# lixinustc/KVQ-Challenge-CVPR-NTIRE2024

Measured on AMD Instinct MI355X. Metric: videos/sec (8-frag x 32 x 224 x 224), higher is better.
Workload: dtype bf16

## Files before the change

### include/kvq_hip.h

```cpp
#ifndef KVQ_HIP_H
#define KVQ_HIP_H

#include <stddef.h>
#include <stdint.h>

#ifdef __cplusplus
extern "C" {
#endif

#define KVQ_ABI_VERSION 31
#define KVQ_MAX_STAGES 4

typedef enum { KVQ_DT_BF16 = 0, KVQ_DT_FP16 = 1 } KvqDtype;

typedef enum {
  KVQ_OK = 0,
  KVQ_ERR_NULL = -1,
  KVQ_ERR_SHAPE = -2,
  KVQ_ERR_UNSUPPORTED = -3,
  KVQ_ERR_WORKSPACE = -4,
  KVQ_ERR_HIP = -5
} KvqStatus;

int kvq_abi_version(void);
// ... 275 lines not shown

int kvq_window_attention(const uint16_t* qkv, const int32_t* tok, const float* rpb, const float* fpb,
                         const float* bias_pack, int table_len, int center, int BW, int nW, int N, int num_heads, int use_mask,
                         int dtype, uint16_t* out, void* stream);

size_t kvq_attn_bias32_bytes(int n_types, int N, int num_heads);
int kvq_attn_bias32_build(const int32_t* tok, const float* rpb, const float* fpb, int table_len, int center,
                          int n_types, int N, int num_heads, int use_mask, void* out, float* max_abs, void* stream);
typedef struct {
  const uint16_t* qkv;
  const void* bias_dense;
  int32_t n_types, BW, nW, N, num_heads, dtype;
  uint16_t* out;
  const uint32_t* tile_skip;
  int32_t dsplit_from;
  const uint16_t* x_ln;
  const uint16_t* w_qkv;
  const float* b_qkv;
  float q_scale;
  const uint32_t* pad_mask;
} KvqAttnDenseArgs;
int kvq_window_attention32(const KvqAttnDenseArgs* host_args, void* stream);
int kvq_window_attention32_ranges(const KvqAttnDenseArgs* host_args, const uint8_t* ranges, void* stream);
int kvq_attn32_row_order(const int32_t* tok_host, int n_windows, int N, int32_t* order);
int kvq_attn32_key_ranges(const int32_t* tok_host, int n_windows, int N, int use_mask, uint8_t* ranges);

int kvq_patch_im2col(const float* x, int B, int Cin, int T, int H, int W, int pd, int ph, int pw,
                     int dtype, uint16_t* out, void* stream);

int kvq_vqa_head(const float* feat, int B, int L, int C, int64_t stride_b, int64_t stride_l,
                 int64_t stride_c, const float* w1t, const float* w1, const float* b1, int hidden, const float* w2,
                 const float* b2, float* scratch, float* score, void* stream);

int kvq_vqa_head_map(const float* feat, int B, int L, int C, int64_t stride_b, int64_t stride_l, int64_t stride_c,
                     const float* w1t, const float* w1, const float* b1, int hidden, const float* w2, const float* b2,
                     int D, float* tok_map, float* depth_score, float* score, void* stream);

typedef struct {
  const KvqFragmentSource* src;
  int32_t T, D, Hf, Wf;
  int32_t cell;
  const float* tok_map;
  float* heat;
  float* cover;
  uint8_t* overlay;
  int32_t ov_depth[16];
  int32_t n_ov;
  const float* range;
// ... 275 lines not shown
```

### kvq-challenge-cvpr-ntire2024_amd/_abi.py

```python
from __future__ import annotations

import ctypes as C
import os
from typing import Optional

from . import _build

MAX_STAGES = 4
K_NAMES = ["im2col", "layernorm", "gemm_qkv", "attn", "gemm_proj", "gemm_fc1", "gemm_fc2", "gemm_merge",
           "gemm_embed", "tail", "embed", "merge"]
K_COUNT = len(K_NAMES)

EPI_BIAS_BF16, EPI_GELU_BF16, EPI_QKV_BF16, EPI_RESID_F32, EPI_STORE_F32, EPI_RELU_BF16, EPI_QGELU_BF16, EPI_RESID_SCALE_F32 = range(8)
DT_BF16, DT_FP16 = 0, 1
ABI_VERSION = 31


def dtype_code(dt) -> int:
    import torch
    is_int = isinstance(dt, int) and not isinstance(dt, bool)
    if (is_int and dt == DT_FP16) or (not is_int and dt in (torch.float16, "fp16", "float16")):
        return DT_FP16
    if (is_int and dt == DT_BF16) or (not is_int and dt in (torch.bfloat16, "bf16", "bfloat16")):
        return DT_BF16
# ... 240 lines not shown
    "kvq_patch_embed_fragments_supported": (i32, [C.POINTER(KvqFragmentSource), i32, i32, i32, i32, i32, i32]),
    "kvq_patch_embed_pack_bytes": (sz, [i32, i32]),
    "kvq_patch_embed_pack": (i32, [p_void, p_void, p_void, p_void, i32, i32, p_void, p_void]),
    "kvq_patch_embed": (i32, [C.POINTER(KvqPatchEmbedArgs), p_void]),
    "kvq_patch_merge_supported": (i32, [i32]),
    "kvq_patch_merge_pack_bytes": (sz, [i32]),
    "kvq_patch_merge_pack": (i32, [p_void, p_void, p_void, i32, i32, p_void, p_void]),
    "kvq_patch_merge": (i32, [C.POINTER(KvqPatchMergeArgs), p_void]),
    "kvq_block_tail_supported": (i32, [i32, i32]),
    "kvq_block_tail_pack_bytes": (sz, [i32, i32]),
    "kvq_block_tail_pack": (i32, [p_void, p_void, p_void, p_void, p_void, p_void, p_void, p_void, i32, i32, p_void,
                                  p_void]),
    "kvq_block_tail_qkv_pack_bytes": (sz, [i32, i32]),
    "kvq_block_tail_qkv_pack": (i32, [p_void, i32, i32, p_void, p_void]),
    "kvq_block_tail": (i32, [C.POINTER(KvqBlockTailArgs), p_void]),
    "kvq_window_attention": (i32, [p_void, p_void, p_void, p_void, p_void, i32, i32, i32, i32, i32, i32, i32, i32, p_void,
                                   p_void]),
    "kvq_attn_bias32_bytes": (sz, [i32, i32, i32]),
    "kvq_attn_bias32_build": (i32, [p_void, p_void, p_void, i32, i32, i32, i32, i32, i32, p_void, p_void, p_void]),
    "kvq_window_attention32": (i32, [C.POINTER(KvqAttnDenseArgs), p_void]),
    "kvq_window_attention32_ranges": (i32, [C.POINTER(KvqAttnDenseArgs), p_void, p_void]),
    "kvq_attn32_row_order": (i32, [p_void, i32, i32, p_void]),
    "kvq_attn32_key_ranges": (i32, [p_void, i32, i32, i32, p_void]),
    "kvq_swin3d_bias_dense_bytes": (sz, [p_void, i32]),
    "kvq_swin3d_bias_dense_build": (i32, [p_void, i32, p_void, p_void, p_void, p_void, p_void]),
    "kvq_patch_im2col": (i32, [p_void, i32, i32, i32, i32, i32, i32, i32, i32, i32, p_void, p_void]),
    "kvq_vqa_head": (i32, [p_void, i32, i32, i32, i64, i64, i64, p_void, p_void, p_void, i32, p_void, p_void, p_void,
                           p_void, p_void]),
    "kvq_vqa_head_map": (i32, [p_void, i32, i32, i32, i64, i64, i64, p_void, p_void, p_void, i32, p_void, p_void, i32, p_void,
                               p_void, p_void, p_void]),
    "kvq_quality_paint_supported": (i32, [C.POINTER(KvqFragmentSource), i32, i32, i32, i32, i32]),
    "kvq_quality_paint": (i32, [C.POINTER(KvqQualityPaintArgs), p_void]),
    "kvq_quality_paint_regions_supported": (i32, [C.POINTER(KvqFragmentSource), i32, i32, i32, i32, i32, i32, i32, i32]),
    "kvq_quality_paint_regions": (i32, [C.POINTER(KvqQualityPaintRegionArgs), p_void]),
    "kvq_vqa_head_classes": (i32, [p_void, i32, i32, i32, i64, i64, i64, p_void, p_void, i32, p_void, p_void, i32, i32, p_void,
                                   p_void, p_void]),
    "kvq_simple_vqa_head": (i32, [p_void, i32, i32, i32, p_void, p_void, i32, p_void, p_void, p_void, p_void,
                                  p_void]),
    "kvq_resize_bilinear": (i32, [p_void, i32, i32, i32, i32, i32, i32, i32, i32, i32, i32, i32, i32, C.POINTER(f32),
                                  C.POINTER(f32), p_void, p_void]),
    "kvq_resize_bilinear_aa": (i32, [p_void, i32, i32, i32, i32, i32, i32, i32, i32, i32, i32, i32, i32, C.POINTER(f32),
                                     C.POINTER(f32), p_void, p_void]),
    "kvq_resize_aa_taps": (i32, [i32, i32, C.POINTER(i32), p_void, p_void, p_void]),
    "kvq_resize_pil_taps": (i32, [i32, i32, C.POINTER(i32), p_void, p_void, p_void]),
    "kvq_resize_pil_supported": (i32, [i32] * 6),
    "kvq_resize_pil": (i32, [p_void, i32, i32, i32, i32, i32, i32, p_void, p_void, p_void, p_void, p_void, p_void, p_void, p_void, i64, i64,
# ... 118 lines not shown
```

### kvq-challenge-cvpr-ntire2024_amd/csrc/attn32.hip

```cpp
#include <stdlib.h>

#include "common.hpp"

#ifndef A32_ABL
#define A32_ABL 0
#endif
#ifndef A32_SUM
#define A32_SUM 0
#endif
#if (A32_ABL & 2)
#define A32_EXP(x) ((x) * 0.001f + 1.0f)
#else
#define A32_EXP(x) __builtin_amdgcn_exp2f(x)
#endif

#ifdef KVQ_DIAG
#define A32_DIAG_FLAG(x) (x)
#else
#define A32_DIAG_FLAG(x) false
#endif

namespace kvq {

constexpr int A32_KB = 13;
// ... 187 lines not shown
      ls = E::dot2(P[cur][i], one2, ls);
      ls1 = E::dot2(P[cur][i + 1], one2, ls1);
    }
#endif
    if (t + 1 < T1) {
      __builtin_amdgcn_sched_group_barrier(0x002, 16, 1);
      __builtin_amdgcn_sched_group_barrier(0x008, 1, 1);
      __builtin_amdgcn_sched_group_barrier(0x002, 12, 1);
      __builtin_amdgcn_sched_group_barrier(0x008, 1, 1);
    }
    __builtin_amdgcn_sched_barrier(0);
  }
  ls += ls1;
  if (A32_SUM == 1) ls = (lv0[0] + lv0[1]) + (lv1[0] + lv1[1]);
  ls = a32_pair_sum(ls);
  a32_finish<E>(O, ls, orow, store);
#undef A32_NR
}

struct Attn32Params {
  const uint16_t* qkv;
  const u32x4* image;
  int BW, nW, N, nH, n_types, qsplit;
  uint16_t* out;
  const uint32_t* tile_skip;
  int dsplit_from;
  const uint8_t* ranges;
  const uint16_t* x_ln;
  const uint16_t* w_qkv;
  const float* b_qkv;
  float q_scale;
  uint16_t* q_out;
  const uint32_t* pad_mask;
  bool no_q_store;
  bool image_one;
};

template <typename E, int KS>
__device__ __forceinline__ void a32_fused_qkv(const Attn32Params& p, unsigned char* slot, int bw, int h, int N) {
  using V8 = typename E::v8;
  const int tid = threadIdx.x, lane = tid & 63, j = lane & 15, g = lane >> 4;
  const int wave = __builtin_amdgcn_readfirstlane(tid >> 6);
  const int C = KS * 32;
  const size_t Mtot = (size_t)p.BW * N;
  const uint16_t* xw = p.x_ln + (size_t)bw * N * C;
  uint16_t* qo = p.q_out + ((size_t)h * Mtot + (size_t)bw * N) * 32;
// ... 49 lines not shown
}

enum { kAllKeys = 0, kDepthSplit = 1, kRanges = 2 };
template <typename E, bool FUSED, int MODE, bool SHORT = false>
__global__ __launch_bounds__(A32_WAVES * 64, 3) __attribute__((amdgpu_waves_per_eu(3, 3))) void window_attention32_kernel(Attn32Params p) {
  fp16_saturate_mode();
  extern __shared__ __attribute__((aligned(16))) unsigned char smem[];
  int* ticket = reinterpret_cast<int*>(smem + A32_OFF_CTR);
  using V8 = typename E::v8;
  const int nclip = p.BW / p.nW, nrep = p.nW / p.n_types, npair = p.n_types * p.nH, per_pair = nclip * nrep * p.qsplit;
  const int xcd = blockIdx.x & 7, slot_i = blockIdx.x >> 3;
  int pair, clip, rep, part;
  if (FUSED) {
    const int per_type = p.nH * nclip * nrep, wt_ = (slot_i / per_type) * 8 + xcd, sub = slot_i % per_type;
    if (wt_ >= p.n_types) return;
    const int h_ = sub % p.nH, rest = sub / p.nH;
    pair = wt_ * p.nH + h_; clip = rest % nclip; rep = rest / nclip; part = 0;
  } else {
    const int sub = slot_i % per_pair;
    pair = (slot_i / per_pair) * 8 + xcd;
    clip = sub % nclip; rep = (sub / nclip) % nrep; part = sub / (nclip * nrep);
  }
  if (pair >= npair) return;
  const int wt = pair / p.nH, h = pair - wt * p.nH, w = rep * p.n_types + wt, bw = clip * p.nW + w;
  const int tid = threadIdx.x, lane = tid & 63, N = p.N, nqb = (N + 31) >> 5;
  const int wave = __builtin_amdgcn_readfirstlane(tid >> 6);
  const size_t Mtot = (size_t)p.BW * N;
  const int C = p.nH * 32;
  const uint16_t* Qg = p.qkv + ((size_t)h * Mtot + (size_t)bw * N) * 32;

  int range_of_lane = 0;
  if (MODE == kRanges) {
    const uint8_t* rg = p.ranges + ((size_t)w * A32_KB + min(lane, A32_KB - 1)) * 2;
    const int first = rg[0], need = (int)rg[1] - first + 1;
    const int len = need <= 4 ? 4 : need <= 7 ? 7 : A32_KB;
    range_of_lane = min(first, A32_KB - len) | (len << 8);
  }
  if (tid < 64) *reinterpret_cast<u32x4*>(smem + A32_OFF_ZERO + tid * 16) = (u32x4){0u, 0u, 0u, 0u};
  if (FUSED) {
    for (int i = tid; i < (A32_ROWS - N) * 8; i += A32_WAVES * 64)
      *reinterpret_cast<u32x4*>(smem + (i & 4 ? A32_K_BYTES : 0) + (N + (i >> 3)) * 64 + (i & 3) * 16) = (u32x4){0u, 0u, 0u, 0u};
    a32_fused_qkv<E, 3>(p, smem, bw, h, N);
  } else {
    const uint16_t* Kg = p.qkv + ((size_t)(1 * p.nH + h) * Mtot + (size_t)bw * N) * 32;
    const uint16_t* Vg = p.qkv + ((size_t)(2 * p.nH + h) * Mtot + (size_t)bw * N) * 32;
    const __amdgpu_buffer_rsrc_t rk = __builtin_amdgcn_make_buffer_rsrc(const_cast<uint16_t*>(Kg), 0, N * 64, 0x00020000);
    const __amdgpu_buffer_rsrc_t rv = __builtin_amdgcn_make_buffer_rsrc(const_cast<uint16_t*>(Vg), 0, N * 64, 0x00020000);
// ... 22 lines not shown
    __syncthreads();
  }

  const int q = lane & 31, hi = lane >> 5;
  const uint32_t skip = p.tile_skip ? p.tile_skip[w] : 0u;
  const bool dsplit = MODE == kDepthSplit && p.dsplit_from >= 0 && w >= p.dsplit_from;
  auto key_range = [&](int qb, int& t0, int& len) __attribute__((always_inline)) {
    t0 = 0; len = A32_KB;
    if (MODE == kDepthSplit && dsplit && qb != 6) { t0 = qb < 6 ? 0 : 6; len = 7; }
    if (MODE == kRanges) {
      const int r = __builtin_amdgcn_readlane(range_of_lane, qb);
      t0 = r & 0xff; len = r >> 8;
    }
  };
  auto take = [&]() -> int {
    int qb_;
    do {
      qb_ = 0;
      if (lane == 0) qb_ = atomicAdd(ticket, 1);
      qb_ = __builtin_amdgcn_readfirstlane(qb_);
    } while (qb_ < q_hi && ((skip >> (2 * qb_)) & 1u) && (((skip >> (2 * qb_ + 1)) & 1u) || 32 * qb_ + 16 >= N));
    return qb_;
  };
  const u32x4* img = p.image + (size_t)(A32_DIAG_FLAG(p.image_one) ? h : pair) * nqb * (A32_KB * 128) + lane;
  struct Req { V8 qf0, qf1; u32x4 pre[2]; int t0, len; };
  auto request = [&](int qb, Req& r) __attribute__((always_inline)) {
    const int qrow = min(32 * qb + q, N - 1);
    r.qf0 = *reinterpret_cast<const V8*>(Qg + (size_t)qrow * 32 + 8 * hi);
    r.qf1 = *reinterpret_cast<const V8*>(Qg + (size_t)qrow * 32 + 16 + 8 * hi);
    if (!FUSED && p.pad_mask && ((p.pad_mask[(size_t)w * A32_KB + qb] >> q) & 1u)) {
      r.qf0 = __builtin_bit_cast(V8, (u32x4){0u, 0u, 0u, 0u});
      r.qf1 = r.qf0;
    }
    key_range(min(qb, nqb - 1), r.t0, r.len);
    const u32x4* bd = img + (size_t)min(qb, nqb - 1) * (A32_KB * 128) + r.t0 * 128;
    r.pre[0] = bd[0]; r.pre[1] = bd[64];
  };
  auto run = [&](int qb, const Req& r) __attribute__((always_inline)) {
    const u32x4* bd = img + (size_t)qb * (A32_KB * 128);
    uint16_t* orow = p.out + ((size_t)bw * N + 32 * qb + q) * C + h * 32;
    const bool store = 32 * qb + q < N;
    const int zero = A32_OFF_ZERO >> 4;
    const int t0 = MODE == kRanges ? r.t0 : 0;
    if (MODE != kAllKeys && r.len == 7) {
      if (r.t0 == A32_KB - 7) a32_qblock<E, 7, true, SHORT>(smem, zero, bd, A32_KB - 7, r.qf0, r.qf1, r.pre, orow, store);
      else a32_qblock<E, 7, false>(smem, zero, bd, t0, r.qf0, r.qf1, r.pre, orow, store);
    } else if (MODE == kRanges && r.len == 4) {
// ... 144 lines not shown
extern "C" int kvq_attn32_key_ranges(const int32_t* tok_host, int n_windows, int N, int use_mask, uint8_t* ranges) {
  using namespace kvq;
  KVQ_REQUIRE(tok_host && ranges, KVQ_ERR_NULL, "kvq_attn32_key_ranges: NULL pointer");
  KVQ_REQUIRE(n_windows > 0 && N >= 1 && N <= 400, KVQ_ERR_SHAPE, "kvq_attn32_key_ranges: bad shape n_windows=%d N=%d", n_windows, N);
  const int nkb = (N + 31) / 32;
  for (int w = 0; w < n_windows; ++w) {
    const int32_t* tk = tok_host + (size_t)w * N * 2;
    for (int qb = 0; qb < A32_KB; ++qb) {
      int first = 0, last = nkb - 1;
      if (use_mask && qb < nkb) {
        bool in_block[256] = {false};
        for (int qq = 32 * qb; qq < N && qq < 32 * qb + 32; ++qq) in_block[(tk[2 * qq + 1] >> 16) & 0xff] = true;
        first = nkb; last = -1;
        for (int key = 0; key < N; ++key)
          if (in_block[(tk[2 * key + 1] >> 16) & 0xff]) { first = first < (key >> 5) ? first : key >> 5; last = key >> 5; }
      }
      ranges[((size_t)w * A32_KB + qb) * 2] = (uint8_t)first;
      ranges[((size_t)w * A32_KB + qb) * 2 + 1] = (uint8_t)last;
    }
  }
  return KVQ_OK;
}

static int window_attention32(const char* who, const KvqAttnDenseArgs* a, const uint8_t* ranges, void* stream) {
  using namespace kvq;
  KVQ_REQUIRE(a && a->qkv && a->bias_dense && a->out, KVQ_ERR_NULL, "%s: NULL pointer", who);
  const int BW = a->BW, nW = a->nW, N = a->N, num_heads = a->num_heads, n_types = a->n_types;
  KVQ_REQUIRE(BW > 0 && nW > 0 && BW % nW == 0 && num_heads > 0 && n_types > 0 && nW % n_types == 0, KVQ_ERR_SHAPE,
              "%s: bad shape BW=%d nW=%d n_types=%d nH=%d", who, BW, nW, n_types, num_heads);
  KVQ_REQUIRE(N >= 1 && N <= 400, KVQ_ERR_UNSUPPORTED, "%s: window of %d tokens unsupported (1..400)", who, N);
  KVQ_REQUIRE(((size_t)a->bias_dense & 15) == 0, KVQ_ERR_SHAPE, "%s: the bias image must be 16-byte aligned", who);
  KVQ_REQUIRE_OPERAND(who, a->dtype);
  KVQ_REQUIRE(a->dsplit_from < 0 || (N == 392 && a->dsplit_from < nW), KVQ_ERR_UNSUPPORTED,
              "%s: depth-split windows need the (8,7,7) window (N = 392); got N=%d from=%d", who, N, a->dsplit_from);
  const int units = BW * num_heads, nqb = (N + 31) / 32;
  int qsplit = units >= 768 ? 1 : 768 / units;
  const int qsplit_max = latency_mode() ? 4 : 1;
  qsplit = qsplit > qsplit_max ? qsplit_max : qsplit;
  qsplit = qsplit > nqb ? nqb : qsplit;
  Attn32Params p{a->qkv, (const u32x4*)a->bias_dense, BW, nW, N, num_heads, n_types, qsplit, a->out, a->tile_skip,
                     a->dsplit_from < 0 ? -1 : a->dsplit_from};
#ifdef KVQ_DIAG
  { static const bool one = getenv("KVQ_IMAGE_ONE_TYPE") && atoi(getenv("KVQ_IMAGE_ONE_TYPE")) == 1; p.image_one = one; }
  { static const bool nq = getenv("KVQ_NO_Q_STORE") && atoi(getenv("KVQ_NO_Q_STORE")) == 1; p.no_q_store = nq; }
#endif
  if (a->pad_mask) {
    KVQ_REQUIRE(a->b_qkv && !a->x_ln, KVQ_ERR_NULL, "%s: pad_mask needs b_qkv (and excludes the fused projection)", who);
    p.pad_mask = a->pad_mask; p.b_qkv = a->b_qkv;
  }
  if (a->x_ln) {
    const int C = 32 * num_heads;
    KVQ_REQUIRE(a->w_qkv && a->b_qkv, KVQ_ERR_NULL, "%s: x_ln without w_qkv / b_qkv", who);
    KVQ_REQUIRE(C == 96, KVQ_ERR_UNSUPPORTED, "%s: the fused qkv projection is built for C = 96 (got %d)", who, C);
    KVQ_REQUIRE((((size_t)a->x_ln | (size_t)a->w_qkv | (size_t)a->b_qkv) & 15) == 0, KVQ_ERR_SHAPE,
                "%s: x_ln / w_qkv / b_qkv must be 16-byte aligned", who);
    p.qsplit = 1;
    p.x_ln = a->x_ln; p.w_qkv = a->w_qkv; p.b_qkv = a->b_qkv; p.q_scale = a->q_scale; p.q_out = const_cast<uint16_t*>(a->qkv);
  }
  if (ranges) {
    KVQ_REQUIRE(a->dsplit_from < 0 && !a->pad_mask, KVQ_ERR_UNSUPPORTED, "%s: key ranges exclude dsplit_from and pad_mask (un-padded partitions only)", who);
    p.ranges = ranges;
  }
  return with_operand(a->dtype, [&](auto e) { return launch_attn32_e<decltype(e)>(p, (hipStream_t)stream); });
}

extern "C" int kvq_window_attention32(const KvqAttnDenseArgs* a, void* stream) {
  return window_attention32("kvq_window_attention32", a, nullptr, stream);
}

extern "C" int kvq_window_attention32_ranges(const KvqAttnDenseArgs* a, const uint8_t* ranges, void* stream) {
  KVQ_REQUIRE(ranges, KVQ_ERR_NULL, "kvq_window_attention32_ranges: NULL ranges");
  return window_attention32("kvq_window_attention32_ranges", a, ranges, stream);
}
```

### kvq-challenge-cvpr-ntire2024_amd/csrc/plan.hip

```cpp
#include <math.h>
#include <stdlib.h>
#include <string.h>

#include <vector>

#include "common.hpp"
#include "tail.hpp"

#ifdef KVQ_DIAG
static int skip_mask() {
  static const int m = [] {
    const int v = getenv("KVQ_SKIP") ? atoi(getenv("KVQ_SKIP")) : 0;
    if (v) fprintf(stderr, "libkvq_hip (KVQ_DIAG build): KVQ_SKIP=%d leaves launch families out - scores are GARBAGE, timing only\n", v);
    return v;
  }();
  return m;
}
#else
static constexpr int skip_mask() { return 0; }
#endif

namespace kvq {

struct StageGeom {
  int D, H, W, C, nH, depth;
  int L;
  int ws[3], ss[3];
  int Dp, Hp, Wp, nW, N, Lp;
  bool shifted_any;
  int32_t* d_src[2];
  int32_t* d_pad[2];
  int32_t* d_skip[2];
  int32_t* d_padmask[2];
  int32_t* d_dst[2];
  int32_t* d_tok[2];
  uint8_t* d_ranges[2];
  int32_t* d_merge;
  int Dn, Hn, Wn;
};

struct ProfEvent {
  int kind, variant;
  double flops, bytes;
  hipEvent_t a, b;
};

}

struct KvqSwinPlan {
  KvqSwinCfg cfg;
  int B, T, H, W, dtype;
  int D0, H0, W0, K0;
  std::vector<kvq::StageGeom> st;
  std::vector<void*> owned;
  size_t ws_bytes;
  size_t off_x0, off_x1, off_ln, off_big, off_o, off_sk, sk_bytes;
  size_t region_bytes[6];
  unsigned char* run_ws;
// ... 116 lines not shown
    if (!pad.empty()) {
      rc = upload(pl, pad, &g.d_pad[par]);
      if (rc) return rc;
      if (g.N <= 13 * 32) {
        std::vector<int32_t> pm((size_t)g.nW * 13, 0);
        for (int i : pad) pm[(size_t)(i / g.N) * 13 + ((i % g.N) >> 5)] |= (int32_t)(1u << ((i % g.N) & 31));
        rc = upload(pl, pm, &g.d_padmask[par]);
        if (rc) return rc;
      }
      std::vector<int32_t> skip((size_t)g.nW, 0);
      bool any = false;
      for (int wv = 0; wv < g.nW; ++wv)
        for (int t = 0; t * 16 < g.N && t < 32; ++t) {
          bool all_pad = true;
          for (int q = t * 16; q < g.N && q < t * 16 + 16; ++q) all_pad = all_pad && src[(size_t)wv * g.N + q] < 0;
          if (all_pad) { skip[wv] |= (int32_t)(1u << t); any = true; }
        }
      if (any) {
        rc = upload(pl, skip, &g.d_skip[par]);
        if (rc) return rc;
      }
    }
  }
  return upload(pl, tok, &g.d_tok[par]);
}

static int build_merge_map(KvqSwinPlan* pl, StageGeom& g) {
  g.Dn = g.D; g.Hn = (g.H + 1) / 2; g.Wn = (g.W + 1) / 2;
  std::vector<int32_t> m((size_t)g.Dn * g.Hn * g.Wn * 4);
  size_t r = 0;
  for (int d = 0; d < g.D; ++d)
    for (int h2 = 0; h2 < g.Hn; ++h2)
      for (int w2 = 0; w2 < g.Wn; ++w2, ++r) {
        const int hh[4] = {2 * h2, 2 * h2 + 1, 2 * h2, 2 * h2 + 1};
        const int wv[4] = {2 * w2, 2 * w2, 2 * w2 + 1, 2 * w2 + 1};
        for (int p = 0; p < 4; ++p)
          m[4 * r + p] = (hh[p] < g.H && wv[p] < g.W) ? (d * g.H + hh[p]) * g.W + wv[p] : -1;
      }
  return upload(pl, m, &g.d_merge);
}

static size_t align_up(size_t v) { return (v + 255) & ~(size_t)255; }

}

extern "C" int kvq_swin3d_plan_create(const KvqSwinCfg* cfg, int B, int T, int H, int W, int dtype,
                                      KvqSwinPlan** out) {
// ... 96 lines not shown
  for (int i = 0; i < pl->cfg.num_stages; ++i) {
    const StageGeom& g = pl->st[i];
    if (block < k + g.depth) {
      *stage = i;
      *par = ((block - k) & 1) && g.shifted_any ? 1 : 0;
      return block >= k;
    }
    k += g.depth;
  }
  return false;
}
}

namespace kvq {
static int bias_types(const StageGeom& g, int par) { return par == 0 ? g.nW / (g.Dp / g.ws[0]) : g.nW; }
constexpr float kQScale = 0.17677669529663687f;
constexpr float kQScaleLog2 = 0.17677669529663687f * 1.4426950408889634f;
}

extern "C" size_t kvq_swin3d_bias_dense_bytes(const KvqSwinPlan* pl, int block) {
  int i = 0, par = 0;
  if (!pl || !kvq::locate_block(pl, block, &i, &par)) return 0;
  const kvq::StageGeom& g = pl->st[i];
  return kvq_attn_bias32_bytes(kvq::bias_types(g, par), g.N, g.nH);
}

extern "C" int kvq_swin3d_bias_dense_build(const KvqSwinPlan* pl, int block, const float* rpb, const float* fpb, void* out,
                                           float* max_abs, void* stream) {
  using namespace kvq;
  int i = 0, par = 0;
  KVQ_REQUIRE(pl && rpb && out, KVQ_ERR_NULL, "kvq_swin3d_bias_dense_build: NULL pointer");
  KVQ_REQUIRE(locate_block(pl, block, &i, &par), KVQ_ERR_SHAPE, "kvq_swin3d_bias_dense_build: no block %d", block);
  const StageGeom& g = pl->st[i];
  return kvq_attn_bias32_build(g.d_tok[par], rpb, pl->cfg.frag_bias[i] ? fpb : nullptr, pl->table_len, pl->center,
                               bias_types(g, par), g.N, g.nH, par, out, max_abs, stream);
}

extern "C" int kvq_swin3d_profile(KvqSwinPlan* pl, int enable) {
  using namespace kvq;
  KVQ_REQUIRE(pl, KVQ_ERR_NULL, "kvq_swin3d_profile: NULL");
  pl->profile = enable != 0;
  pl->ev_used = 0;
  return KVQ_OK;
}

extern "C" int kvq_swin3d_profile_read(KvqSwinPlan* pl, KvqProfRecord* out, int max_records, int* n_records) {
  using namespace kvq;
  KVQ_REQUIRE(pl && out && n_records, KVQ_ERR_NULL, "kvq_swin3d_profile_read: NULL");
  int n = 0;
  for (size_t i = 0; i < pl->ev_used && n < max_records; ++i, ++n) {
    ProfEvent& e = pl->events[i];
    KVQ_CHECK_HIP(hipEventSynchronize(e.b));
    float t = 0.f;
    KVQ_CHECK_HIP(hipEventElapsedTime(&t, e.a, e.b));
    out[n].kind = e.kind; out[n].variant = e.variant; out[n].ms = t; out[n].flops = e.flops; out[n].bytes = e.bytes;
  }
  *n_records = n;
  pl->ev_used = 0;
// ... 196 lines not shown
    const int C = g.C;
    const float qs = bw.bias_dense ? kQScaleLog2 : kQScale;
    if (t.ln1 != kFromProducer)
      KVQ_TRY(ln(pl, st, cur, t.ln1 == kLnTokens ? nullptr : g.d_src[t.par], 1, g.L, t.ln1 == kLnTokens ? g.L : g.Lp, C, bw.norm1_w,
                 bw.norm1_b, bln, nullptr, s.x16[t.i]));
    if (t.qkv == kQkvGemm)
      KVQ_TRY_UNLESS(8 | (t.i == last ? 32 : 0), gemm(pl, st, KVQ_K_GEMM_QKV, bln, bw.qkv_w, bw.qkv_b, B * g.Lp, 3 * C, C, KVQ_EPI_QKV_BF16, bbig, nullptr, g.nH, qs));
    if (t.qkv == kQkvGemmPadded)
      KVQ_TRY(gemm(pl, st, KVQ_K_GEMM_QKV, bln, bw.qkv_w, bw.qkv_b, B * g.L, 3 * C, C, KVQ_EPI_QKV_BF16, bbig, nullptr, g.nH,
                   qs, g.d_dst[t.par], g.L, g.Lp));
    if (t.fill_pad) KVQ_TRY(kvq_qkv_fill_pad(bbig, bw.qkv_b, g.d_pad[t.par], g.Lp - g.L, B, g.Lp, g.nH, qs, pl->dtype, st));
    return KVQ_OK;
  };

  auto attention = [&](const BlockStep& t, const StageGeom& g, const KvqSwinBlockW& bw) -> int {
    const int C = g.C, M = B * g.Lp;
    if (!t.dense) {
      Bracket br(pl, st, KVQ_K_ATTN, (cfg.frag_bias[t.i] ? 2 : 0) + t.par, 4.0 * M * g.N * C, 2.0 * 4.0 * M * C);
      return kvq_window_attention(bbig, g.d_tok[t.par], bw.rpb_table, cfg.frag_bias[t.i] ? bw.fpb_table : nullptr, bw.bias_pack,
                                  pl->table_len, pl->center, B * g.nW, g.nW, g.N, g.nH, t.par, pl->dtype, bo, st);
    }
    const bool fq = t.qkv == kQkvInAttn;
    Bracket br(pl, st, KVQ_K_ATTN, 4 + t.par, 4.0 * M * g.N * C + (fq ? 6.0 * M * C * C : 0.0),
               (fq ? 2.0 * 2.0 * M * C + 6.0 * C * C : 2.0 * 4.0 * M * C) + (double)kvq_swin3d_bias_dense_bytes(pl, t.blk));
    KvqAttnDenseArgs aa{};
    aa.qkv = bbig; aa.bias_dense = bw.bias_dense; aa.n_types = bias_types(g, t.par); aa.BW = B * g.nW; aa.nW = g.nW; aa.N = g.N;
    aa.num_heads = g.nH; aa.dtype = pl->dtype; aa.out = bo; aa.tile_skip = (const uint32_t*)g.d_skip[t.par]; aa.dsplit_from = t.dsplit_from;
    if (fq) { aa.x_ln = bln; aa.w_qkv = bw.qkv_w; aa.b_qkv = bw.qkv_b; aa.q_scale = kQScaleLog2; }
    if (t.pad_mask) { aa.pad_mask = (const uint32_t*)g.d_padmask[t.par]; aa.b_qkv = bw.qkv_b; }
    if (g.d_ranges[t.par]) KVQ_TRY_UNLESS(1 | (t.i == last ? 32 : 0), kvq_window_attention32_ranges(&aa, g.d_ranges[t.par], st));
    else KVQ_TRY_UNLESS(1 | (t.i == last ? 32 : 0), kvq_window_attention32(&aa, st));
    return KVQ_OK;
  };

  auto tail = [&](const BlockStep& t, const StageGeom& g, const KvqSwinBlockW& bw) -> int {
    const int C = g.C, M = B * g.Lp, ML = B * g.L, hidden = cfg.mlp_ratio * C, skip_last = t.i == last ? 32 : 0;
    if (t.fused_tail) {
      const bool e1 = t.emit == kEmitLn1, eq = t.emit == kEmitQkv, x16 = s.x16[t.i];
      KvqBlockTailArgs ta{};
      ta.attn = bo; ta.x = cur; ta.scatter_map = g.d_src[t.par]; ta.map_rows = g.Lp; ta.out_rows = g.L;
      ta.M = M; ta.C = C; ta.hidden = hidden; ta.pack = bw.tail_pack; ta.eps = 1e-5f; ta.dtype = pl->dtype; ta.x_f16 = x16 ? 1 : 0;
      if (g.Lp != g.L) ta.attn_gather = g.d_dst[t.par];
      if (t.emit != kEmitNone) {
        const KvqSwinBlockW& nb = w->blocks[t.blk + 1];
        ta.next_norm_w = nb.norm1_w; ta.next_norm_b = nb.norm1_b; ta.next_dst = g.d_dst[t.npar]; ta.next_rows = g.Lp;
        if (eq) { ta.next_qkv_pack = nb.qkv_pack; ta.next_qkv_b = nb.qkv_b; ta.qkv_out = bbig; ta.q_scale = kQScaleLog2; ta.num_heads = g.nH; }
        else ta.next_ln = bln;
      }
      Bracket br(pl, st, KVQ_K_TAIL, kvq::tailmm_geometry_code(C, hidden) * 1000 + (C / 32) * 10 + t.emit, 2.0 * M * C * C + 4.0 * (double)ML * C * hidden + (eq ? 6.0 * M * C * C : 0.0),
                 (double)M * C * 2.0 + (double)ML * C * ((x16 ? 4.0 : 8.0) + (e1 ? 2.0 : 0.0) + (eq ? 6.0 : 0.0)));
      KVQ_TRY_UNLESS(C <= 192 ? 2 : 4, block_tail_launch(&ta, range_of(t.i), st));
      return KVQ_OK;
    }
    if (g.Lp != g.L) {
// ... 117 lines not shown
```

### kvq-challenge-cvpr-ntire2024_amd/kernels.py

```python
from __future__ import annotations

import ctypes as C
from typing import Optional, Sequence

import torch

from . import _abi
from ._abi import check, current_stream, dtype_code, lib, ptr, stream_of
from ._prepared import to_operand

HALF_TYPES = (torch.float16, torch.bfloat16)


def _need_gpu(*ts):
    for t in ts:
        if t is not None and not t.is_cuda:
            raise _abi.KvqError("kvq_amd kernels need tensors on a HIP device (no CPU fallback exists)")


def device_name() -> str:
    buf = C.create_string_buffer(256)
    check(lib().kvq_device_name(buf, 256), "kvq_device_name")
    return buf.value.decode()

# ... 156 lines not shown
    check(lib().kvq_window_attention(ptr(qkv), ptr(tok), ptr(rpb), ptr(fpb), ptr(bias_pack), rpb.shape[0], center, BW, nW, N, nH,
                                     int(use_mask), dtype_code(qkv.dtype), ptr(out), current_stream()),
          "kvq_window_attention")
    return out


LOG2E = 1.4426950408889634


def attn_bias32(tok: torch.Tensor, rpb: torch.Tensor, fpb: Optional[torch.Tensor], center: int, nW: int, N: int, use_mask: bool):
    _need_gpu(tok, rpb, fpb)
    nH = rpb.shape[1]
    out = torch.empty(lib().kvq_attn_bias32_bytes(nW, N, nH), dtype=torch.uint8, device=rpb.device)
    big = torch.zeros(1, dtype=torch.float32, device=rpb.device)
    check(lib().kvq_attn_bias32_build(ptr(tok), ptr(rpb), ptr(fpb), rpb.shape[0], center, nW, N, nH, int(use_mask),
                                      ptr(out), ptr(big), current_stream()), "kvq_attn_bias32_build")
    out.max_abs_bias = big
    return out


def window_attention32(qkv: torch.Tensor, image: torch.Tensor, nW: int, N: int, n_types: Optional[int] = None,
                       tile_skip: Optional[torch.Tensor] = None, out: Optional[torch.Tensor] = None, dsplit_from: int = -1,
                       x_ln: Optional[torch.Tensor] = None, w_qkv: Optional[torch.Tensor] = None, b_qkv: Optional[torch.Tensor] = None,
                       q_scale: float = 1.0, pad_mask: Optional[torch.Tensor] = None, ranges: Optional[torch.Tensor] = None):
    _need_gpu(qkv, image, tile_skip, out, pad_mask, ranges)
    assert qkv.dtype in HALF_TYPES and qkv.is_contiguous()
    nH = qkv.shape[1]
    BW = qkv.shape[2] // N
    if out is None:
        out = torch.empty(BW * N, nH * 32, dtype=qkv.dtype, device=qkv.device)
    a = _abi.KvqAttnDenseArgs()
    a.qkv, a.bias_dense, a.n_types, a.BW, a.nW, a.N, a.num_heads = ptr(qkv), ptr(image), nW if n_types is None else n_types, BW, nW, N, nH
    a.dtype, a.out, a.tile_skip, a.dsplit_from = dtype_code(qkv.dtype), ptr(out), ptr(tile_skip), dsplit_from
    if x_ln is not None:
        _need_gpu(x_ln, w_qkv, b_qkv)
        assert x_ln.dtype == qkv.dtype == w_qkv.dtype and x_ln.is_contiguous() and w_qkv.is_contiguous() and b_qkv.dtype == torch.float32
        a.x_ln, a.w_qkv, a.b_qkv, a.q_scale = ptr(x_ln), ptr(w_qkv), ptr(b_qkv), q_scale
    if pad_mask is not None:
        _need_gpu(b_qkv)
        assert pad_mask.dtype == torch.int32 and pad_mask.is_contiguous() and (b_qkv is None or b_qkv.dtype == torch.float32)
        a.pad_mask, a.b_qkv = ptr(pad_mask), ptr(b_qkv)
    if ranges is not None:
        assert ranges.dtype == torch.uint8 and ranges.is_contiguous() and ranges.numel() == nW * 26
        check(lib().kvq_window_attention32_ranges(C.byref(a), ptr(ranges), current_stream()), "kvq_window_attention32_ranges")
        return out
    check(lib().kvq_window_attention32(C.byref(a), current_stream()), "kvq_window_attention32")
    return out


def attn32_row_order(tok, n_windows: int, N: int):
    import numpy as np
    tok = np.ascontiguousarray(np.asarray(tok, dtype=np.int32).reshape(n_windows * N, 2))
    order = np.empty((n_windows, N), np.int32)
    check(lib().kvq_attn32_row_order(tok.ctypes.data, n_windows, N, order.ctypes.data), "kvq_attn32_row_order")
    return order


def attn32_key_ranges(tok, n_windows: int, N: int, use_mask: bool):
    import numpy as np
    tok = np.ascontiguousarray(np.asarray(tok, dtype=np.int32).reshape(n_windows * N, 2))
    ranges = np.empty((n_windows, 13, 2), np.uint8)
    check(lib().kvq_attn32_key_ranges(tok.ctypes.data, n_windows, N, int(use_mask), ranges.ctypes.data), "kvq_attn32_key_ranges")
    return ranges


def patch_im2col(x: torch.Tensor, patch: Sequence[int], out_dtype=torch.float16):
    _need_gpu(x)
    assert x.dtype == torch.float32 and x.is_contiguous()
    B, Cin, T, H, W = x.shape
    pd, ph, pw = patch
    D, Hh, Ww = -(-T // pd), -(-H // ph), -(-W // pw)
    out = torch.empty(B * D * Hh * Ww, Cin * pd * ph * pw, dtype=out_dtype, device=x.device)
    check(lib().kvq_patch_im2col(ptr(x), B, Cin, T, H, W, pd, ph, pw, dtype_code(out_dtype), ptr(out),
                                 current_stream()), "kvq_patch_im2col")
    return out


def vqa_head(feat: torch.Tensor, w1, b1, w2, b2, w1t=None, return_map=False):
    _need_gpu(feat, w1, b1, w2, b2, w1t)
    assert feat.dtype == torch.float32 and feat.dim() == 5
    B, Cc, D, H, W = feat.shape
    L = D * H * W
    sb, sc, sd, sh, sw = feat.stride()
    if not (sh == W * sw and sd == H * sh):
        feat = feat.contiguous()
        sb, sc, sd, sh, sw = feat.stride()
# ... 1301 lines not shown
```

Baseline: 439.5.

## Deduplicate identical attention bias images across window types and balance slot order

At plan time, window types whose token-to-bias key patterns are identical after normalising the fragment offset are grouped, so the dense attention bias image is built and stored only once per distinct pattern. A type table maps each work pair to its real window type and canonical image, and duplicated types are interleaved across eight slots so that blocks sharing an image are spread out. This shrinks the bias buffer and the memory traffic and cache footprint it causes in the attention kernel. The cost is one extra table load per block and more complex host-side planning.

```diff
diff --git a/include/kvq_hip.h b/include/kvq_hip.h
--- a/include/kvq_hip.h
+++ b/include/kvq_hip.h
@@ -321,8 +321,10 @@
 } KvqAttnDenseArgs;
 int kvq_window_attention32(const KvqAttnDenseArgs* host_args, void* stream);
 int kvq_window_attention32_ranges(const KvqAttnDenseArgs* host_args, const uint8_t* ranges, void* stream);
+int kvq_window_attention32_types(const KvqAttnDenseArgs* host_args, const uint8_t* ranges, const int32_t* type_tab, void* stream);
 int kvq_attn32_row_order(const int32_t* tok_host, int n_windows, int N, int32_t* order);
 int kvq_attn32_key_ranges(const int32_t* tok_host, int n_windows, int N, int use_mask, uint8_t* ranges);
+int kvq_attn32_image_types(const int32_t* tok_host, int n_types, int N, int32_t* canon, int32_t* slots, int32_t* n_images);
 
 int kvq_patch_im2col(const float* x, int B, int Cin, int T, int H, int W, int pd, int ph, int pw,
                      int dtype, uint16_t* out, void* stream);
diff --git a/kvq-challenge-cvpr-ntire2024_amd/_abi.py b/kvq-challenge-cvpr-ntire2024_amd/_abi.py
--- a/kvq-challenge-cvpr-ntire2024_amd/_abi.py
+++ b/kvq-challenge-cvpr-ntire2024_amd/_abi.py
@@ -286,6 +286,8 @@
     "kvq_window_attention32_ranges": (i32, [C.POINTER(KvqAttnDenseArgs), p_void, p_void]),
     "kvq_attn32_row_order": (i32, [p_void, i32, i32, p_void]),
     "kvq_attn32_key_ranges": (i32, [p_void, i32, i32, i32, p_void]),
+    "kvq_window_attention32_types": (i32, [C.POINTER(KvqAttnDenseArgs), p_void, p_void, p_void]),
+    "kvq_attn32_image_types": (i32, [p_void, i32, i32, p_void, p_void, p_void]),
     "kvq_swin3d_bias_dense_bytes": (sz, [p_void, i32]),
     "kvq_swin3d_bias_dense_build": (i32, [p_void, i32, p_void, p_void, p_void, p_void, p_void]),
     "kvq_patch_im2col": (i32, [p_void, i32, i32, i32, i32, i32, i32, i32, i32, i32, p_void, p_void]),
diff --git a/kvq-challenge-cvpr-ntire2024_amd/csrc/attn32.hip b/kvq-challenge-cvpr-ntire2024_amd/csrc/attn32.hip
--- a/kvq-challenge-cvpr-ntire2024_amd/csrc/attn32.hip
+++ b/kvq-challenge-cvpr-ntire2024_amd/csrc/attn32.hip
@@ -1,4 +1,8 @@
 #include <stdlib.h>
+
+#include <algorithm>
+#include <map>
+#include <vector>
 
 #include "common.hpp"
 
@@ -233,6 +237,7 @@
   const uint16_t* qkv;
   const u32x4* image;
   int BW, nW, N, nH, n_types, qsplit;
+  const int32_t* type_tab;
   uint16_t* out;
   const uint32_t* tile_skip;
   int dsplit_from;
@@ -328,7 +333,10 @@
     clip = sub % nclip; rep = (sub / nclip) % nrep; part = sub / (nclip * nrep);
   }
   if (pair >= npair) return;
-  const int wt = pair / p.nH, h = pair - wt * p.nH, w = rep * p.n_types + wt, bw = clip * p.nW + w;
+  const int wp = pair / p.nH, h = pair - wp * p.nH;
+  int wt = wp, im = wp;
+  if (p.type_tab) { const int e = p.type_tab[wp]; wt = e & 0xffff; im = e >> 16; }
+  const int w = rep * p.n_types + wt, bw = clip * p.nW + w;
   const int tid = threadIdx.x, lane = tid & 63, N = p.N, nqb = (N + 31) >> 5;
   const int wave = __builtin_amdgcn_readfirstlane(tid >> 6);
   const size_t Mtot = (size_t)p.BW * N;
@@ -397,7 +405,7 @@
     } while (qb_ < q_hi && ((skip >> (2 * qb_)) & 1u) && (((skip >> (2 * qb_ + 1)) & 1u) || 32 * qb_ + 16 >= N));
     return qb_;
   };
-  const u32x4* img = p.image + (size_t)(A32_DIAG_FLAG(p.image_one) ? h : pair) * nqb * (A32_KB * 128) + lane;
+  const u32x4* img = p.image + (size_t)(A32_DIAG_FLAG(p.image_one) ? h : im * p.nH + h) * nqb * (A32_KB * 128) + lane;
   struct Req { V8 qf0, qf1; u32x4 pre[2]; int t0, len; };
   auto request = [&](int qb, Req& r) __attribute__((always_inline)) {
     const int qrow = min(32 * qb + q, N - 1);
@@ -588,7 +596,42 @@
   return KVQ_OK;
 }
 
-static int window_attention32(const char* who, const KvqAttnDenseArgs* a, const uint8_t* ranges, void* stream) {
+extern "C" int kvq_attn32_image_types(const int32_t* tok_host, int n_types, int N, int32_t* canon, int32_t* slots, int32_t* n_images) {
+  KVQ_REQUIRE(tok_host && canon && slots && n_images, KVQ_ERR_NULL, "kvq_attn32_image_types: NULL pointer");
+  KVQ_REQUIRE(n_types > 0 && N >= 1, KVQ_ERR_SHAPE, "kvq_attn32_image_types: bad shape n_types=%d N=%d", n_types, N);
+  std::map<std::vector<int32_t>, int> seen;
+  std::vector<std::vector<int>> members;
+  std::vector<int32_t> key((size_t)N * 2);
+  for (int t = 0; t < n_types; ++t) {
+    const int32_t* tk = tok_host + (size_t)t * N * 2;
+    int fh0 = 255, fw0 = 255;
+    for (int n = 0; n < N; ++n) { fh0 = std::min(fh0, tk[2 * n + 1] & 0xff); fw0 = std::min(fw0, (tk[2 * n + 1] >> 8) & 0xff); }
+    for (int n = 0; n < N; ++n) { key[2 * n] = tk[2 * n]; key[2 * n + 1] = tk[2 * n + 1] - fh0 - (fw0 << 8); }
+    const auto it = seen.emplace(key, (int)members.size());
+    if (it.second) members.emplace_back();
+    canon[t] = it.first->second;
+    members[canon[t]].push_back(t);
+  }
+  *n_images = (int32_t)members.size();
+  for (int t = 0; t < n_types; ++t) slots[t] = t;
+  if ((int)members.size() == n_types) return KVQ_OK;
+  std::vector<int> by_size(members.size());
+  for (size_t i = 0; i < by_size.size(); ++i) by_size[i] = (int)i;
+  std::stable_sort(by_size.begin(), by_size.end(), [&](int a, int b) { return members[a].size() > members[b].size(); });
+  int room[8], fill[8] = {0};
+  for (int c = 0; c < 8; ++c) room[c] = n_types > c ? (n_types - c + 7) / 8 : 0;
+  for (int gi : by_size) {
+    const std::vector<int>& m = members[gi];
+    for (size_t k = 0; k < m.size();) {
+      int c = 0;
+      for (int o = 1; o < 8; ++o) if (room[o] - fill[o] > room[c] - fill[c]) c = o;
+      for (; k < m.size() && fill[c] < room[c]; ++k) slots[c + 8 * fill[c]++] = m[k];
+    }
+  }
+  return KVQ_OK;
+}
+
+static int window_attention32(const char* who, const KvqAttnDenseArgs* a, const uint8_t* ranges, const int32_t* type_tab, void* stream) {
   using namespace kvq;
   KVQ_REQUIRE(a && a->qkv && a->bias_dense && a->out, KVQ_ERR_NULL, "%s: NULL pointer", who);
   const int BW = a->BW, nW = a->nW, N = a->N, num_heads = a->num_heads, n_types = a->n_types;
@@ -604,7 +647,7 @@
   const int qsplit_max = latency_mode() ? 4 : 1;
   qsplit = qsplit > qsplit_max ? qsplit_max : qsplit;
   qsplit = qsplit > nqb ? nqb : qsplit;
-  Attn32Params p{a->qkv, (const u32x4*)a->bias_dense, BW, nW, N, num_heads, n_types, qsplit, a->out, a->tile_skip,
+  Attn32Params p{a->qkv, (const u32x4*)a->bias_dense, BW, nW, N, num_heads, n_types, qsplit, type_tab, a->out, a->tile_skip,
                      a->dsplit_from < 0 ? -1 : a->dsplit_from};
 #ifdef KVQ_DIAG
   { static const bool one = getenv("KVQ_IMAGE_ONE_TYPE") && atoi(getenv("KVQ_IMAGE_ONE_TYPE")) == 1; p.image_one = one; }
@@ -631,10 +674,14 @@
 }
 
 extern "C" int kvq_window_attention32(const KvqAttnDenseArgs* a, void* stream) {
-  return window_attention32("kvq_window_attention32", a, nullptr, stream);
+  return window_attention32("kvq_window_attention32", a, nullptr, nullptr, stream);
 }
 
 extern "C" int kvq_window_attention32_ranges(const KvqAttnDenseArgs* a, const uint8_t* ranges, void* stream) {
   KVQ_REQUIRE(ranges, KVQ_ERR_NULL, "kvq_window_attention32_ranges: NULL ranges");
-  return window_attention32("kvq_window_attention32_ranges", a, ranges, stream);
-}
+  return window_attention32("kvq_window_attention32_ranges", a, ranges, nullptr, stream);
+}
+
+extern "C" int kvq_window_attention32_types(const KvqAttnDenseArgs* a, const uint8_t* ranges, const int32_t* type_tab, void* stream) {
+  return window_attention32("kvq_window_attention32_types", a, ranges, type_tab, stream);
+}
diff --git a/kvq-challenge-cvpr-ntire2024_amd/csrc/plan.hip b/kvq-challenge-cvpr-ntire2024_amd/csrc/plan.hip
--- a/kvq-challenge-cvpr-ntire2024_amd/csrc/plan.hip
+++ b/kvq-challenge-cvpr-ntire2024_amd/csrc/plan.hip
@@ -34,6 +34,9 @@
   int32_t* d_padmask[2];
   int32_t* d_dst[2];
   int32_t* d_tok[2];
+  int n_images[2];
+  int32_t* d_tok_img[2];
+  int32_t* d_type_tab[2];
   uint8_t* d_ranges[2];
   int32_t* d_merge;
   int Dn, Hn, Wn;
@@ -196,7 +199,25 @@
       }
     }
   }
-  return upload(pl, tok, &g.d_tok[par]);
+  rc = upload(pl, tok, &g.d_tok[par]);
+  if (rc) return rc;
+  const int types = par == 0 ? g.nW / nd : g.nW;
+  std::vector<int32_t> canon((size_t)types), slots((size_t)types);
+  int32_t n_images = types;
+  rc = kvq_attn32_image_types(tok.data(), types, g.N, canon.data(), slots.data(), &n_images);
+  if (rc) return rc;
+  g.n_images[par] = types; g.d_tok_img[par] = g.d_tok[par]; g.d_type_tab[par] = nullptr;
+  if (n_images < types && types <= 0xffff) {
+    std::vector<int32_t> tok_img((size_t)n_images * g.N * 2), tab((size_t)types);
+    for (int t = types - 1; t >= 0; --t)
+      memcpy(&tok_img[(size_t)canon[t] * g.N * 2], &tok[(size_t)t * g.N * 2], (size_t)g.N * 2 * sizeof(int32_t));
+    for (int p = 0; p < types; ++p) tab[p] = slots[p] | (canon[slots[p]] << 16);
+    rc = upload(pl, tok_img, &g.d_tok_img[par]);
+    if (!rc) rc = upload(pl, tab, &g.d_type_tab[par]);
+    if (rc) return rc;
+    g.n_images[par] = n_images;
+  }
+  return KVQ_OK;
 }
 
 static int build_merge_map(KvqSwinPlan* pl, StageGeom& g) {
@@ -339,7 +360,7 @@
   int i = 0, par = 0;
   if (!pl || !kvq::locate_block(pl, block, &i, &par)) return 0;
   const kvq::StageGeom& g = pl->st[i];
-  return kvq_attn_bias32_bytes(kvq::bias_types(g, par), g.N, g.nH);
+  return kvq_attn_bias32_bytes(g.n_images[par], g.N, g.nH);
 }
 
 extern "C" int kvq_swin3d_bias_dense_build(const KvqSwinPlan* pl, int block, const float* rpb, const float* fpb, void* out,
@@ -349,8 +370,8 @@
   KVQ_REQUIRE(pl && rpb && out, KVQ_ERR_NULL, "kvq_swin3d_bias_dense_build: NULL pointer");
   KVQ_REQUIRE(locate_block(pl, block, &i, &par), KVQ_ERR_SHAPE, "kvq_swin3d_bias_dense_build: no block %d", block);
   const StageGeom& g = pl->st[i];
-  return kvq_attn_bias32_build(g.d_tok[par], rpb, pl->cfg.frag_bias[i] ? fpb : nullptr, pl->table_len, pl->center,
-                               bias_types(g, par), g.N, g.nH, par, out, max_abs, stream);
+  return kvq_attn_bias32_build(g.d_tok_img[par], rpb, pl->cfg.frag_bias[i] ? fpb : nullptr, pl->table_len, pl->center,
+                               g.n_images[par], g.N, g.nH, par, out, max_abs, stream);
 }
 
 extern "C" int kvq_swin3d_profile(KvqSwinPlan* pl, int enable) {
@@ -593,14 +614,13 @@
     }
     const bool fq = t.qkv == kQkvInAttn;
     Bracket br(pl, st, KVQ_K_ATTN, 4 + t.par, 4.0 * M * g.N * C + (fq ? 6.0 * M * C * C : 0.0),
-               (fq ? 2.0 * 2.0 * M * C + 6.0 * C * C : 2.0 * 4.0 * M * C) + (double)kvq_swin3d_bias_dense_bytes(pl, t.blk));
+               (fq ? 2.0 * 2.0 * M * C + 6.0 * C * C : 2.0 * 4.0 * M * C) + (double)kvq_attn_bias32_bytes(bias_types(g, t.par), g.N, g.nH));
     KvqAttnDenseArgs aa{};
     aa.qkv = bbig; aa.bias_dense = bw.bias_dense; aa.n_types = bias_types(g, t.par); aa.BW = B * g.nW; aa.nW = g.nW; aa.N = g.N;
     aa.num_heads = g.nH; aa.dtype = pl->dtype; aa.out = bo; aa.tile_skip = (const uint32_t*)g.d_skip[t.par]; aa.dsplit_from = t.dsplit_from;
     if (fq) { aa.x_ln = bln; aa.w_qkv = bw.qkv_w; aa.b_qkv = bw.qkv_b; aa.q_scale = kQScaleLog2; }
     if (t.pad_mask) { aa.pad_mask = (const uint32_t*)g.d_padmask[t.par]; aa.b_qkv = bw.qkv_b; }
-    if (g.d_ranges[t.par]) KVQ_TRY_UNLESS(1 | (t.i == last ? 32 : 0), kvq_window_attention32_ranges(&aa, g.d_ranges[t.par], st));
-    else KVQ_TRY_UNLESS(1 | (t.i == last ? 32 : 0), kvq_window_attention32(&aa, st));
+    KVQ_TRY_UNLESS(1 | (t.i == last ? 32 : 0), kvq_window_attention32_types(&aa, g.d_ranges[t.par], g.d_type_tab[t.par], st));
     return KVQ_OK;
   };
 
diff --git a/kvq-challenge-cvpr-ntire2024_amd/kernels.py b/kvq-challenge-cvpr-ntire2024_amd/kernels.py
--- a/kvq-challenge-cvpr-ntire2024_amd/kernels.py
+++ b/kvq-challenge-cvpr-ntire2024_amd/kernels.py
@@ -202,8 +202,9 @@
 def window_attention32(qkv: torch.Tensor, image: torch.Tensor, nW: int, N: int, n_types: Optional[int] = None,
                        tile_skip: Optional[torch.Tensor] = None, out: Optional[torch.Tensor] = None, dsplit_from: int = -1,
                        x_ln: Optional[torch.Tensor] = None, w_qkv: Optional[torch.Tensor] = None, b_qkv: Optional[torch.Tensor] = None,
-                       q_scale: float = 1.0, pad_mask: Optional[torch.Tensor] = None, ranges: Optional[torch.Tensor] = None):
-    _need_gpu(qkv, image, tile_skip, out, pad_mask, ranges)
+                       q_scale: float = 1.0, pad_mask: Optional[torch.Tensor] = None, ranges: Optional[torch.Tensor] = None,
+                       type_tab: Optional[torch.Tensor] = None):
+    _need_gpu(qkv, image, tile_skip, out, pad_mask, ranges, type_tab)
     assert qkv.dtype in HALF_TYPES and qkv.is_contiguous()
     nH = qkv.shape[1]
     BW = qkv.shape[2] // N
@@ -222,6 +223,11 @@
         a.pad_mask, a.b_qkv = ptr(pad_mask), ptr(b_qkv)
     if ranges is not None:
         assert ranges.dtype == torch.uint8 and ranges.is_contiguous() and ranges.numel() == nW * 26
+    if type_tab is not None:
+        assert type_tab.dtype == torch.int32 and type_tab.is_contiguous() and type_tab.numel() == a.n_types
+        check(lib().kvq_window_attention32_types(C.byref(a), ptr(ranges), ptr(type_tab), current_stream()), "kvq_window_attention32_types")
+        return out
+    if ranges is not None:
         check(lib().kvq_window_attention32_ranges(C.byref(a), ptr(ranges), current_stream()), "kvq_window_attention32_ranges")
         return out
     check(lib().kvq_window_attention32(C.byref(a), current_stream()), "kvq_window_attention32")
@@ -242,6 +248,14 @@
     ranges = np.empty((n_windows, 13, 2), np.uint8)
     check(lib().kvq_attn32_key_ranges(tok.ctypes.data, n_windows, N, int(use_mask), ranges.ctypes.data), "kvq_attn32_key_ranges")
     return ranges
+
+
+def attn32_image_types(tok, n_types: int, N: int):
+    import numpy as np
+    tok = np.ascontiguousarray(np.asarray(tok, dtype=np.int32).reshape(n_types * N, 2))
+    canon, slots, n = np.empty(n_types, np.int32), np.empty(n_types, np.int32), C.c_int32(0)
+    check(lib().kvq_attn32_image_types(tok.ctypes.data, n_types, N, canon.ctypes.data, slots.ctypes.data, C.addressof(n)), "kvq_attn32_image_types")
+    return canon, slots, int(n.value)
 
 
 def patch_im2col(x: torch.Tensor, patch: Sequence[int], out_dtype=torch.float16):
```

Result: slower. 434.4 (-1.2%).
